# bark-simulator/planner-miqp

Measured on AMD Instinct MI355X. Metric: MIQP solves/sec to 1% gap, 2-agent x 20-step x 32-region, higher is better.
Workload: dtype f64

## Files before the change

planner_miqp_amd/csrc/kernels.hip:

```cpp
#include <hip/hip_runtime.h>

#include "host_inst.hpp"

#ifndef MIQP_RHO
#define MIQP_RHO 1.0e5
#endif

#ifndef MIQP_IPM_WPE
#define MIQP_IPM_WPE 3
#endif

#ifdef MIQP_ABLATE
#define MIQP_ABL (B.abl)
#else
#define MIQP_ABL 0
#endif
namespace miqp {

constexpr double RHO_EL = MIQP_RHO;
constexpr double FEAS_TOL = 1.0e-6;
constexpr double QP_TOL = 1.0e-6;
#ifndef MIQP_T0
#define MIQP_T0 1.0e-3
#endif
// ... 1937 lines not shown
    int nk = 0, nfar = 0, nnear = 0; double fmin_ = 1e300;
    for (int a = 0; a < nalt; ++a) {
      const double cb = objlb + clift[a];
      if (inc_now < 1e300 && (inc_now - cb) <= gapi * (1e-10 + fabs(inc_now))) { if (B.stats) atomicAdd(&B.stats[56], 1ull); continue; }
      int negm = 0;
      if (chosen.kind == 3 && ck[a] >= 0 && ck[a] < N && (B.seq_kinds & 0x10000) == 0) {
        negm = 1 << (int)comp[base + ck[a] * stride];
        for (int a2 = 1; a2 < a; ++a2) if (ck[a2] == ck[a]) negm |= 1 << ca[a2];
      }
      const bool tf = (cb - cst) > thr && B.batch_depth[node] != REPAIR_ROOT;
      k_ck[nk] = ck[a]; k_ca[nk] = ca[a]; k_neg[nk] = negm; k_ord[nk] = a; k_bnd[nk] = cb - cst;
      k_pos[nk] = tf ? (0x40000000 | nfar++) : nnear++;
      if (tf) fmin_ = fmin(fmin_, cb - cst);
      nk++;
    }
    int fbase = 0, obase = 0, ob2 = 0, extra2 = 0; bool okalloc = true;
    if (nnear > 0) {
      obase = atomicAdd(&B.open_count[inst], nnear);
      if (obase + nnear > B.open_cap) {
        for (int q = obase; q < obase + nnear && q < B.open_cap; ++q) { size_t oi = ((size_t)B.open_sel * B.n_slots + slot) * B.open_cap + q; B.open_bound[oi] = 1e300; B.open_node[oi] = -1; B.open_depth[oi] = 0; }
        if (B.far_cap > 0) { for (int q = 0; q < nk; ++q) if (!(k_pos[q] & 0x40000000)) { k_pos[q] = 0x40000000 | nfar++; fmin_ = fmin(fmin_, k_bnd[q]); } }
        else okalloc = false;
        nnear = 0; obase = 0;
      }
    }
    const int nnear_kept = nnear;
    if (nfar > 0) {
      fbase = atomicAdd(&B.far_count[inst], nfar);
      if (fbase + nfar <= B.far_cap) atomicMin(&B.far_minkey[inst], d2key(fmin_));
      else {
        for (int q = fbase; q < fbase + nfar && q < B.far_cap; ++q) { B.far_bound[(size_t)slot * B.far_cap + q] = 1e300; B.far_node[(size_t)slot * B.far_cap + q] = -1; }
        int extra = 0;
        for (int q = 0; q < nk; ++q) if (k_pos[q] & 0x40000000) k_pos[q] = 0x20000000 | extra++;
        nfar = 0;
        ob2 = atomicAdd(&B.open_count[inst], extra); extra2 = extra;
        if (ob2 + extra > B.open_cap) {
          okalloc = false;
          for (int q = ob2; q < ob2 + extra && q < B.open_cap; ++q) { size_t oi = ((size_t)B.open_sel * B.n_slots + slot) * B.open_cap + q; B.open_bound[oi] = 1e300; B.open_node[oi] = -1; B.open_depth[oi] = 0; }
        }
        sh_base[3] = ob2;
      }
    }
    if (okalloc && nk > 0) {
      unsigned int h = atomicAdd(B.free_head, (unsigned int)nk);
      if ((int)(*B.free_limit - h) >= nk) {
        for (int q = 0; q < nk; ++q) slots[q] = B.free_q[(h + q) % (unsigned int)B.pool_cap];
      } else {
        int nb = atomicAdd(B.pool_count, nk);
        if (nb + nk > B.pool_cap) okalloc = false;
        for (int q = 0; q < nk; ++q) slots[q] = nb + q;
      }
    }
    if (!okalloc) {
      atomicOr(&B.inst_flags[inst], 1);
      for (int q = fbase; q < fbase + nfar; ++q) { B.far_bound[(size_t)slot * B.far_cap + q] = 1e300; B.far_node[(size_t)slot * B.far_cap + q] = -1; }
      for (int q = obase; q < obase + nnear_kept && q < B.open_cap; ++q) { size_t oi = ((size_t)B.open_sel * B.n_slots + slot) * B.open_cap + q; B.open_bound[oi] = 1e300; B.open_node[oi] = -1; B.open_depth[oi] = 0; }
      for (int q = ob2; q < ob2 + extra2 && q < B.open_cap; ++q) { size_t oi = ((size_t)B.open_sel * B.n_slots + slot) * B.open_cap + q; B.open_bound[oi] = 1e300; B.open_node[oi] = -1; B.open_depth[oi] = 0; }
      nk = 0;
    }
    if (B.stats && nk > 0) { atomicAdd(&B.stats[43], 1ull); atomicAdd(&B.stats[44], (unsigned long long)nk); atomicAdd(&B.stats[48 + chosen.kind], 1ull); atomicAdd(&B.stats[52 + chosen.kind], (unsigned long long)nk); }
    sh_base[0] = fbase; sh_base[1] = obase; sh_base[2] = nk;
  }
  __syncthreads();
  PROF_T(te5);
  const int nk = sh_base[2];
  if (nk <= 0) { FREE_NODE(); return; }
  {
    for (int q = 0; q < nk; ++q) {
      signed char* dst = B.pool_fix + (size_t)slots[q] * Y.fixlen;
      const int kk = k_ck[q]; const signed char av = (signed char)k_ca[q];
      int negidx = -1; const int negm = k_neg[q];
      if (chosen.kind == 3 && kk >= 0 && kk < N && (B.seq_kinds & 0x10000) == 0) negidx = Y.f_c2n + (chosen.c * N + kk) * 4 + chosen.o;
      if (kk != -2) {
        for (int k8 = lane; k8 < Y.fixlen / 8; k8 += 64) ((unsigned long long*)cfix)[k8] = ((const unsigned long long*)fix)[k8];
        __syncthreads();
        for (int j = jlo + lane; j <= jhi; j += 64) { const int k = base + j * stride; if (fix[k] < 0) { if (j < kk) cfix[k] = comp[k]; else if (j == kk) cfix[k] = av; } }
        __syncthreads();
        if (lane == 0 && negidx >= 0) cfix[negidx] = (signed char)negm;
        __syncthreads();
        for (int k8 = lane; k8 < Y.fixlen / 8; k8 += 64) ((unsigned long long*)dst)[k8] = ((const unsigned long long*)cfix)[k8];
        __syncthreads();
      } else
      for (int k = lane; k < Y.fixlen; k += 64) {
        signed char v = fix[k];
        int rel = k - base;
        if (v < 0 && rel >= 0 && rel % stride == 0) {
          int j = rel / stride;
          if (j >= jlo && j <= jhi) { if (j < kk) v = comp[k]; else if (j == kk) v = av; }
        }
        if (k == negidx) v = (signed char)negm;
        if (kk == -2) {
          v = (fix[k] < 0 && k < Y.f_c2n) ? comp[k] : fix[k];
          if ((B.opt2 & 0x10000) && fix[k] < 0 && k >= Y.f_env && k < Y.f_c2c && (k - Y.f_env) % 5 != 0) v = fix[k];
          if (B.probe_margin > 0.0 && fix[k] < 0 && ploose[k]) v = fix[k];
        }
        dst[k] = v;
      }
      if (B.pool_origin && lane == 0) {
        int cls = k_ord[q] > 0 ? 1 : 0;
        if (chosen.kind == 0 && cls) { const int rq = (int)comp[base + chosen.i * stride] >> 2, cq = k_ca[q] >> 2; const int dq = T[Y.i_regj + chosen.c * P + cq] - T[Y.i_regj + chosen.c * P + rq]; const int ad = abs(dq) % Y.R;
          cls = (k_ca[q] & 3) == 3 ? 3 : ((ad == 1 || ad == Y.R - 1) ? 1 : 2); }
        B.pool_origin[slots[q]] = (signed char)(kk == -2 ? 15 : 4 * chosen.kind + cls);
      }
    }
    if (B.pool_big && lane < nk) B.pool_big[slots[lane]] = pumped ? (unsigned char)((((big_parent >> 4) + 1) << 4) | 1) : (unsigned char)(big_parent & ~12);
    if (B.pool_Z) {
      for (int q = 0; q < nk; ++q) { if (slots[q] >= B.z_cap) continue; double* zd = B.pool_Z + (size_t)slots[q] * N * NZ; for (int k = lane; k < N * NZ; k += 64) zd[k] = Z[k]; }
    }
    if (B.pool_A) {
      const bool as_node = B.batch_A && B.batch_large && B.batch_large[node] <= 1;
      const unsigned short av_ = as_node ? B.batch_A[(size_t)node * 64 + lane] : (unsigned short)0xFFFFu;
      for (int q = 0; q < nk; ++q) { if (slots[q] >= B.z_cap) continue; B.pool_A[(size_t)slots[q] * 64 + lane] = av_; }
      if (B.ring_M && lane < nk && slots[lane] < B.z_cap) B.pool_Mtag[slots[lane]] = as_node ? B.batch_Mtag[node] : 0ull;
    }
    if (lane < nk) {
      int pd = B.batch_depth[node] >> 6;
      int pref = k_ord[lane];
      if (B.opt2 & 2) {
        pref = 0;
        for (int q = 0; q < nk; ++q) if (k_bnd[q] < k_bnd[lane] || (k_bnd[q] == k_bnd[lane] && q < lane)) pref++;
      }
      const int dw = k_ck[lane] == -2 ? (((pd + 2) << 6) | 63) : (((pd + 1) << 6) | (62 - (pref < 62 ? pref : 62)));
      if (k_pos[lane] & 0x40000000) {
        size_t oi = (size_t)slot * B.far_cap + sh_base[0] + (k_pos[lane] & 0x3FFFFFFF);
        B.far_bound[oi] = k_bnd[lane]; B.far_node[oi] = slots[lane]; B.far_depth[oi] = dw;
      } else {
        const int np_ = (k_pos[lane] & 0x20000000) ? sh_base[3] + (k_pos[lane] & 0x1FFFFFFF) : sh_base[1] + k_pos[lane];
        size_t oi = ((size_t)B.open_sel * B.n_slots + slot) * B.open_cap + np_;
        B.open_bound[oi] = k_bnd[lane]; B.open_node[oi] = slots[lane]; B.open_depth[oi] = dw;
      }
    }
  }
  FREE_NODE();
#ifdef MIQP_PROFILE
  { PROF_T(te6);
    if (lane == 0) { atomicAdd(&B.prof[100], (unsigned long long)(te1 - te0)); atomicAdd(&B.prof[101], (unsigned long long)(te2 - te1)); atomicAdd(&B.prof[102], (unsigned long long)(te3 - te2));
                     atomicAdd(&B.prof[103], (unsigned long long)(te4 - te3)); atomicAdd(&B.prof[104], (unsigned long long)(te5 - te4)); atomicAdd(&B.prof[105], (unsigned long long)(te6 - te5)); atomicAdd(&B.prof[106], 1ull); } }
#endif
#undef FREE_NODE
}

constexpr int SEL_THREADS = 1024;
constexpr int SEL_LOWSHIFT = 24;

__device__ inline int wave_append(int* counter, bool pred) {
  const unsigned long long mk = __ballot(pred);
  const int lane = threadIdx.x & 63;
  int base = 0;
  if (lane == (int)(__ffsll((long long)mk) - 1)) base = atomicAdd(counter, __popcll(mk));
  base = __shfl(base, mk ? (int)(__ffsll((long long)mk) - 1) : 0);
  return base + __popcll(mk & ((1ull << lane) - 1ull));
}

__global__ void __launch_bounds__(SEL_THREADS) select_kernel(DevBuf B, int round) {
  const Layout& Y = B.Y;
  const int slot = blockIdx.x, tid = threadIdx.x;
#ifdef MIQP_PROFILE
  if (slot == 0 && tid == 0) {
    const unsigned long long a = B.prof[120], b = B.prof[121], c = B.prof[122];
    if (b != 0 && a != ~0ull && a != 0) { B.prof[123] += b - a; B.prof[124] += b - c; B.prof[125] += 1; }
    B.prof[120] = ~0ull; B.prof[121] = 0; B.prof[122] = ~0ull;
  }
#endif
  const int inst = B.slot_inst[slot];
  if (inst < 0 || B.inst_done[inst] || B.inst_kill[inst]) { if (tid == 0) B.slot_demand[slot] = 0; }
  if (inst < 0) return;
  const int cap = B.open_cap;
  __shared__ int sh_take, sh_base, sh_m, sh_keep, sh_pick, sh_ties, sh_w, sh_mv, sh_all, sh_elig;
  __shared__ double sh_inc;
  __shared__ unsigned int hist[256], dhist[256], sh_wsum[4];
  __shared__ int sh_bin;
  __shared__ int sh_dkeep, sh_tiecnt, sh_ndef;
  __shared__ unsigned long long sh_thr2;
  __shared__ unsigned long long sh_prefix, sh_thr, sh_fmin;
  __shared__ double red[SEL_THREADS];
  if (B.inst_done[inst]) return;
  const size_t src = ((size_t)B.open_sel * B.n_slots + slot) * cap, dst = ((size_t)(1 - B.open_sel) * B.n_slots + slot) * cap;
  unsigned long long* keys = B.open_key + (size_t)slot * cap;
  PROF_T(ts0);
  if (tid == 0) {
    unsigned long long key = B.inc_key[inst];
    sh_inc = inc_from_key(key);
    sh_take = -1;
    sh_thr = key != B.inc_seen[inst] ? key : ~0ull;
    sh_fmin = ~0ull;
    sh_m = 0; sh_keep = 0; sh_pick = 0; sh_ties = 0; sh_ndef = 0;
  }
  __syncthreads();
  if (sh_thr != ~0ull) {
    const unsigned long long key = sh_thr;
    const int pbc = B.prev_bc < B.batch_cap ? B.prev_bc : B.batch_cap;
    for (int k = tid; k < pbc; k += SEL_THREADS) if (B.batch_candkey[k] == key && B.batch_candinst[k] == inst) atomicMin(&sh_fmin, d2key(B.batch_obj[k]));
    __syncthreads();
    const unsigned long long bo = sh_fmin;
    if (tid == 0) sh_dkeep = 0x7FFFFFFF;
    __syncthreads();
    if (bo != ~0ull) for (int k = tid; k < pbc; k += SEL_THREADS) if (B.batch_candkey[k] == key && B.batch_candinst[k] == inst && d2key(B.batch_obj[k]) == bo) atomicMin(&sh_dkeep, k);
    __syncthreads();
    if (tid == 0 && sh_dkeep != 0x7FFFFFFF) { sh_take = sh_dkeep; B.inc_seen[inst] = key; }
  }
  __syncthreads();
  if (sh_take >= 0) {
    const int bslot = sh_take;
    const signed char* cf = B.batch_comp + (size_t)bslot * Y.fixlen; signed char* df = B.inc_fix + (size_t)inst * Y.fixlen;
    for (int k = tid; k < Y.fixlen; k += SEL_THREADS) df[k] = cf[k];
    const double* zs = B.batch_Z + (size_t)bslot * Y.N * Y.nz; double* zd = B.inc_Z + (size_t)inst * Y.N * Y.nz;
    for (int k = tid; k < Y.N * Y.nz; k += SEL_THREADS) zd[k] = zs[k];
    if (B.inc_A && B.batch_A && B.batch_Mtag) {
      if (tid < 64) B.inc_A[(size_t)inst * 64 + tid] = B.batch_A[(size_t)bslot * 64 + tid];
      if (tid == 0) B.inc_Mtag[inst] = B.batch_Mtag[bslot];
    }
    if (tid == 0) { B.inc_obj[inst] = B.batch_obj[bslot]; if (B.inst_lns) B.inst_lns[inst] |= 1; }
  }
  __syncthreads();
  if (B.inst_kill[inst]) {
    int nn = B.open_count[inst]; if (nn > cap) nn = cap;
    for (int k = tid; k < nn; k += SEL_THREADS) { const int nd = B.open_node[src + k]; if (nd >= 0) { unsigned int q_ = atomicAdd(B.free_tail, 1u); B.free_q[q_ % (unsigned int)B.pool_cap] = nd; } }
    int fn = B.far_cap > 0 ? B.far_count[inst] : 0; if (fn > B.far_cap) fn = B.far_cap;
    for (int k = tid; k < fn; k += SEL_THREADS) { const int nd = B.far_node[(size_t)slot * (size_t)B.far_cap + k]; if (nd >= 0) { unsigned int q_ = atomicAdd(B.free_tail, 1u); B.free_q[q_ % (unsigned int)B.pool_cap] = nd; } }
    __syncthreads();
    if (tid == 0) {
      B.open_count[inst] = 0; if (B.far_cap > 0) B.far_count[inst] = 0;
      atomicOr(&B.inst_flags[inst], 2); B.inst_done[inst] = 1; atomicSub(B.active_insts, 1);
    }
    return;
  }
  PROF_T(ts1);
  const double inc = fmin(sh_inc < 1e300 ? B.inc_obj[inst] : 1e300, B.inc_ext[inst]);
  const double cst = B.inst_const[inst];
  const double gap = B.inst_gap[inst];
  int n = B.open_count[inst]; if (n > cap) n = cap;
  auto prunable = [&](double b) { return inc < 1e300 && (inc - (b + cst)) <= gap * (1e-10 + fabs(inc)); };
  auto radix = [&](auto keyf, int cnt, int need) -> int {
    if (tid == 0) { sh_prefix = 0ull; sh_all = 0; }
    __syncthreads();
    for (int shift = 56; shift >= SEL_LOWSHIFT; shift -= 8) {
      if (tid < 256) hist[tid] = 0u;
      __syncthreads();
      const unsigned long long prefix = sh_prefix;
      const unsigned long long himask = shift == 56 ? 0ull : (~0ull << (shift + 8));
      for (int k = tid; k < cnt; k += SEL_THREADS) {
        unsigned long long key = keyf(k);
        if (key != ~0ull && (key & himask) == prefix) atomicAdd(&hist[(key >> shift) & 255ull], 1u);
      }
      __syncthreads();
      if (tid == 0) sh_bin = 256;
      unsigned int hv = 0, hx = 0;
      if (tid < 256) {
        hv = hist[tid]; hx = hv;
#pragma unroll
        for (int o = 1; o < 64; o <<= 1) { const unsigned int y = __shfl_up(hx, o); if ((tid & 63) >= o) hx += y; }
        if ((tid & 63) == 63) sh_wsum[tid >> 6] = hx;
      }
      __syncthreads();
      if (tid < 256) {
#pragma unroll
        for (int w = 0; w < 3; ++w) if (w < (tid >> 6)) hx += sh_wsum[w];
        if (hx >= (unsigned int)need) atomicMin(&sh_bin, tid);
        if (tid == 255) sh_wsum[3] = hx;
      }
      __syncthreads();
      {
        const int bin0 = sh_bin;
        if (tid == (bin0 < 256 ? bin0 : 255)) {
          const int bin = bin0 < 256 ? bin0 : 255;
          const unsigned int cum = bin0 < 256 ? hx - hv : sh_wsum[3];
          if (bin0 >= 256 && shift == 56) sh_all = 1;
          sh_prefix = prefix | ((unsigned long long)bin << shift);
          sh_pick = need - (int)cum;
          sh_tiecnt = (int)hv;
        }
      }
      __syncthreads();
      need = sh_pick;
      if (sh_all) break;
    }
    __syncthreads();
    return need;
  };
  const unsigned long long lowmask = (1ull << SEL_LOWSHIFT) - 1ull;
  int keep = cap / 4; { const int k2 = 2 * B.batch_cap > 65536 ? 2 * B.batch_cap : 65536; if (keep > k2) keep = k2; }
  const int spill_at = 2 * keep;
  const size_t fb = (size_t)slot * (size_t)B.far_cap;
  int fc = B.far_cap > 0 ? B.far_count[inst] : 0; if (fc > B.far_cap) fc = B.far_cap;
  const int dive_every = (B.seq_kinds >> 18) & 3;
  const bool periodic = dive_every == 0 ? (round & 3) == 3 : (dive_every == 1 ? false : (dive_every == 2 ? (round & 7) == 7 : (round & 1) == 1));
  bool pool_tight;
  { const int pc = *B.pool_count; const long long live = (long long)(pc < B.pool_cap ? pc : B.pool_cap) - (long long)(int)(*B.free_tail - *B.free_head);
    pool_tight = live > (long long)B.pool_cap / 10 * 9; }
  const bool lists_full = B.far_cap > 0 ? fc > B.far_cap / 4 * 3 : n > cap / 2;
  const bool dive = !(inc < 1e300) || periodic || lists_full || pool_tight;
  auto order_key = [&](double b, int dp) -> unsigned long long {
    const int dbias = (B.seq_kinds >> 24) & 3;
    const double bb = dbias ? b - (dbias == 1 ? 1e-4 : (dbias == 2 ? 1e-3 : 1e-2)) * fabs(b) * (double)(dp >> 6) : b;
    if (dive) { const unsigned long long kd = ((unsigned long long)(0xFFFF - (dp < 0xFFFF ? dp : 0xFFFF)) << 48) | (d2key(fmax(b, -1e300)) >> 16); return kd == ~0ull ? ~0ull - 1 : kd; }
    const double kv = fmax(bb, -1e300);
    const unsigned long long key = d2key(kv); return key == ~0ull ? ~0ull - 1 : key;
  };
  PROF_T(ts2);
  for (int k = tid; k < 256; k += SEL_THREADS) dhist[k] = 0u;
  __syncthreads();
  double lb = 1e300; int mloc = 0, ndef = 0;
  const bool big_round = B.probe_every <= 1 || (round % B.probe_every) == B.probe_every - 1;
  for (int k = tid; k < n; k += SEL_THREADS) {
    double b = B.open_bound[src + k]; int nd = B.open_node[src + k]; int dp = B.open_depth[src + k];
    unsigned long long key = ~0ull;
    if (nd < 0) { keys[k] = key; continue; }
    if (prunable(b)) {
      unsigned int q_ = atomicAdd(B.free_tail, 1u); B.free_q[q_ % (unsigned int)B.pool_cap] = nd;
    } else {
      lb = fmin(lb, b);
      key = order_key(b, dp);
      if (!big_round && is_probe_word(dp)) { key = ~0ull - 1; ndef++; }
      atomicAdd(&dhist[(dp >> 6) > 255 ? 255 : (dp >> 6)], 1u);
      mloc++;
    }
    keys[k] = key;
  }
  if (mloc) atomicAdd(&sh_m, mloc);
  if (ndef) atomicAdd(&sh_ndef, ndef);
  __syncthreads();
  int m = sh_m;
  PROF_T(ts3);
  if (fc > 0 && m < keep / 4 && cap - n >= 64) {
    auto fkey = [&](int k) -> unsigned long long {
      const double b = B.far_bound[fb + k];
      if (B.far_node[fb + k] < 0 || prunable(b)) return ~0ull;
      const unsigned long long key = d2key(b); return key == ~0ull ? ~0ull - 1 : key;
    };
    int stride = fc > 4 * keep ? (fc + keep - 1) / keep : 1;
    if (stride > 1 && (fc + stride - 1) / stride > cap - n) stride = (fc + (cap - n) - 1) / (cap - n);
    if (stride > 1) {
      const int ns = (fc + stride - 1) / stride;
      for (int j = tid; j < ns; j += SEL_THREADS) keys[n + j] = fkey(j * stride);
      __syncthreads();
      int need_s = (keep - m) / stride; if (need_s < 1) need_s = 1;
      radix([&](int k) { return keys[n + k]; }, ns, need_s);
    } else radix(fkey, fc, keep - m);
    const unsigned long long thr = sh_all ? ~0ull : sh_prefix;
    if (tid == 0) { sh_w = 0; sh_mv = 0; sh_fmin = ~0ull; }
    __syncthreads();
    int room = cap - n; if (room > keep - m) room = keep - m; if (room < 0) room = 0;
    constexpr int PER = 4;
    for (int c0 = 0; c0 < fc; c0 += SEL_THREADS * PER) {
      double eb[PER]; int en[PER], ed[PER], act[PER];
#pragma unroll
      for (int j = 0; j < PER; ++j) {
        const int k = c0 + j * SEL_THREADS + tid;
        act[j] = -1;
        if (k < fc) {
          eb[j] = B.far_bound[fb + k]; en[j] = B.far_node[fb + k]; ed[j] = B.far_depth[fb + k];
          if (en[j] < 0) act[j] = -1;
          else if (prunable(eb[j])) act[j] = 0;
          else { unsigned long long key = d2key(eb[j]); if (key == ~0ull) key = ~0ull - 1; act[j] = ((key & ~lowmask) <= thr) ? 2 : 1; }
        }
      }
      __syncthreads();
#pragma unroll
      for (int j = 0; j < PER; ++j) {
        if (act[j] == 0) { unsigned int q_ = atomicAdd(B.free_tail, 1u); B.free_q[q_ % (unsigned int)B.pool_cap] = en[j]; }
        int t = wave_append(&sh_mv, act[j] == 2);
        if (act[j] == 2) {
          if (t < room) {
            B.open_bound[src + n + t] = eb[j]; B.open_node[src + n + t] = en[j]; B.open_depth[src + n + t] = ed[j]; keys[n + t] = order_key(eb[j], ed[j]);
            lb = fmin(lb, eb[j]); atomicAdd(&dhist[(ed[j] >> 6) > 255 ? 255 : (ed[j] >> 6)], 1u);
          } else act[j] = 1;
        }
        int pos = wave_append(&sh_w, act[j] == 1);
        if (act[j] == 1) { B.far_bound[fb + pos] = eb[j]; B.far_node[fb + pos] = en[j]; B.far_depth[fb + pos] = ed[j]; atomicMin(&sh_fmin, d2key(eb[j])); }
      }
      __syncthreads();
    }
    const int moved = sh_mv < room ? sh_mv : room;
    n += moved; m += moved;
    fc = sh_w;
    __syncthreads();
    if (tid == 0) {
      B.far_count[inst] = fc; B.far_minkey[inst] = sh_fmin;
      B.near_thr[inst] = (fc > 0 && thr != ~0ull) ? key2d(thr | lowmask) : 1e300;
    }
  }
  PROF_T(ts4);
  lb = wave_min(lb);
  __syncthreads();
  if ((tid & 63) == 0) red[tid >> 6] = lb;
  __syncthreads();
#pragma unroll
  for (int w = 0; w < SEL_THREADS / 64; ++w) lb = fmin(lb, red[w]);
  if (fc > 0) lb = fmin(lb, key2d(B.far_minkey[inst]));
  const bool spill = B.far_cap > 0 && m > spill_at && fc < B.far_cap;
  unsigned long long thr_spill = ~0ull;
  if (spill) {
    radix([&](int k) { return keys[k]; }, n, keep);
    thr_spill = sh_all ? ~0ull : sh_prefix;
    if (tid == 0) { unsigned int cum = 0; int d = 255; for (; d >= 0; --d) { if (cum + dhist[d] > (unsigned int)(keep / 2)) break; cum += dhist[d]; } sh_dkeep = d + 1; }
    __syncthreads();
  }
  const int dkeep = sh_dkeep;
  PROF_T(ts5);
  if (tid == 0) sh_pick = 0;
  __syncthreads();
  const int act_now = *B.active_insts;
  const int focus_at = 16 << ((B.seq_kinds >> 29) & 3);
  const bool focus = act_now <= focus_at && inc < 1e300 && (B.seq_kinds & 0x8000000) == 0;
  if (focus) {
    const double gme = (inc - (lb + cst)) / (1e-10 + fabs(inc));
    int cntl = 0;
    for (int sj = tid; sj < B.n_slots; sj += SEL_THREADS) {
      const int j = B.slot_inst[sj];
      if (j < 0 || j == inst || B.inst_done[j]) continue;
      const double ij = B.inc_obj[j];
      const double gj = ij < 1e299 ? (ij - B.lower_bound[j]) / (1e-10 + fabs(ij)) : 1e300;
      if (gj < gme || (gj == gme && j < inst)) cntl++;
    }
    if (cntl) atomicAdd(&sh_pick, cntl);
  }
  __syncthreads();
  const int rank = sh_pick;
  __syncthreads();
  int m_elig = m - sh_ndef;
  if (!dive && inc < 1e300 && B.window_pct < 100 && m > 0) {
    const double top = inc - gap * (1e-10 + fabs(inc)) - cst;
    const double thrw = lb + 0.01 * (double)B.window_pct * fmax(0.0, top - lb);
    const unsigned long long kw = d2key(thrw);
    if (tid == 0) sh_elig = 0;
    __syncthreads();
    int ce = 0;
    for (int k = tid; k < n; k += SEL_THREADS) { const unsigned long long key = keys[k]; if (key != ~0ull && key <= kw) ce++; }
    if (ce) atomicAdd(&sh_elig, ce);
    __syncthreads();
    m_elig = sh_elig < 1 ? 1 : sh_elig;
    if (m_elig > m - sh_ndef) m_elig = m - sh_ndef;
  }
  if (tid == 0) {
    sh_pick = 0;
    int act = act_now; if (act < 1) act = 1;
    int w;
    if (B.seq_kinds & 0x40000000) {
      w = (focus && !(B.seq_kinds & 0x10000000)) ? (B.batch_cap >> (rank + 1 < 30 ? rank + 1 : 30)) : B.batch_cap / act;
      if (w < B.nodes_per_round) w = B.nodes_per_round;
    } else { w = B.slot_take[slot]; if (w < B.base_take && !(B.young_nodes > 0 && B.inst_nodes[inst] >= (long long)B.young_nodes)) w = B.base_take; }
    if (B.width_cap > 0 && w > B.width_cap) w = B.width_cap;
    if (!(inc < 1e300) && w > 512) w = 512;
    if (B.lns_narrow > 0 && B.inst_lns && (B.inst_lns[inst] & 1) && inc < 1e300 && B.inst_nodes[inst] >= (long long)B.lns_min_nodes && w > B.lns_narrow) w = B.lns_narrow;
    B.slot_demand[slot] = inc < 1e300 ? m_elig : (m < 512 ? m : 512);
    int take = m_elig < w ? m_elig : w;
    const int maxch = B.far_cap > 0 ? 8 : 64;
    int room = (cap - m) / maxch; if (room < 1) room = 1;
    if (B.far_cap > 0 && room < 1024) room = 1024;
    if (take > room) take = room;
    int base = take > 0 ? atomicAdd(B.batch_count, take) : 0;
    if (base + take > B.batch_cap) take = B.batch_cap > base ? B.batch_cap - base : 0;
    sh_take = take; sh_base = base;
    double lbt = ((n > 0 || fc > 0) && lb < 1e300 ? lb + cst : inc);
    if (inc < 1e300 && lbt > inc) lbt = inc;
    B.lower_bound[inst] = lbt;
    if (m == 0 && fc == 0) { B.inst_done[inst] = 1; atomicSub(B.active_insts, 1); }
    B.inst_mode[inst] = dive ? 1 : 0;
    sh_thr = ~0ull; sh_w = fc; sh_fmin = ~0ull;
  }
  __syncthreads();
  PROF_T(ts6);
  const int take = sh_take, base = sh_base;
  auto second_key = [&](unsigned long long key, int dp) -> unsigned long long { return (((key & lowmask) << 6) | (unsigned long long)(63 - (dp & 63))) << 34; };
  if (take > 0 && take < m) {
    int need = radix([&](int k) { return keys[k]; }, n, take);
    const unsigned long long thr1 = sh_prefix; const int tiecnt = sh_tiecnt;
    __syncthreads();
    unsigned long long thr2 = ~0ull;
    if (B.det_ties && need < tiecnt) {
      if (tiecnt <= SEL_THREADS) {
        unsigned long long* tie = (unsigned long long*)red;
        if (tid == 0) sh_elig = 0;
        __syncthreads();
        for (int k = tid; k < n; k += SEL_THREADS) {
          const unsigned long long key = keys[k];
          if (key != ~0ull && (key & ~lowmask) == thr1) { const int t = atomicAdd(&sh_elig, 1); if (t < SEL_THREADS) tie[t] = second_key(key, B.open_depth[src + k]); }
        }
        __syncthreads();
        const int tc = sh_elig < SEL_THREADS ? sh_elig : SEL_THREADS;
        if (tid < tc) {
          const unsigned long long v = tie[tid]; int lt = 0, le = 0;
          for (int j = 0; j < tc; ++j) { const unsigned long long u = tie[j]; lt += u < v ? 1 : 0; le += u <= v ? 1 : 0; }
          if (lt < need && need <= le) { sh_thr2 = v; sh_ties = need - lt; }
        }
        __syncthreads();
        thr2 = sh_thr2; need = sh_ties;
        __syncthreads();
      } else {
        need = radix([&](int k) -> unsigned long long { const unsigned long long key = keys[k]; if (key == ~0ull || (key & ~lowmask) != thr1) return ~0ull; return second_key(key, B.open_depth[src + k]); }, n, need);
        thr2 = sh_prefix;
        __syncthreads();
      }
    }
    if (tid == 0) { sh_thr = thr1; sh_thr2 = thr2; sh_ties = need; sh_pick = 0; }
    __syncthreads();
  } else if (tid == 0) { sh_thr = take >= m ? ~0ull : 0ull;    sh_thr2 = ~0ull; sh_ties = 0x7FFFFFFF; sh_pick = 0; }
  __syncthreads();
  PROF_T(ts7);
  const unsigned long long thr = sh_thr, thr2 = sh_thr2;
  for (int k0 = 0; k0 < n; k0 += SEL_THREADS) {
    const int k = k0 + tid;
    unsigned long long key = k < n ? keys[k] : ~0ull;
    const bool live = key != ~0ull;
    double b = 0.0; int nd = 0, dp = 0;
    bool pick = false;
    if (live) {
      b = B.open_bound[src + k]; nd = B.open_node[src + k]; dp = B.open_depth[src + k];
      if (take > 0) {
        const unsigned long long kh = key & (~0ull << SEL_LOWSHIFT);
        if (kh < thr) pick = true;
        else if (kh == thr) {
          const unsigned long long s2 = thr2 != ~0ull ? second_key(key, dp) : 0ull;
          if (thr2 != ~0ull && s2 < thr2) pick = true;
          else if (thr2 == ~0ull || s2 == thr2) { int t = atomicAdd(&sh_ties, -1); pick = t > 0; }
        }
      }
      if (pick) {
        int pos = atomicAdd(&sh_pick, 1);
        if (pos < take) { B.batch_node[base + pos] = nd; B.batch_inst[base + pos] = inst; B.batch_bound[base + pos] = b; B.batch_depth[base + pos] = dp;
                          if (B.batch_large) { const int lc_ = large_class(B, nd, dp, inc < 1e300); B.batch_large[base + pos] = (unsigned char)lc_;
                            if (lc_ && B.cls_list) { const int q_ = atomicAdd(&B.cls_count[lc_ - 1], 1); if (q_ < B.batch_cap) B.cls_list[(size_t)(lc_ - 1) * B.batch_cap + q_] = base + pos; } } }
        else pick = false;
      }
    }
    bool tofar = live && !pick && spill && (key & ~lowmask) > thr_spill && (dp >> 6) < dkeep;
    int fpos = wave_append(&sh_w, tofar);
    if (tofar) {
      if (fpos < B.far_cap) { B.far_bound[fb + fpos] = b; B.far_node[fb + fpos] = nd; B.far_depth[fb + fpos] = dp; atomicMin(&sh_fmin, d2key(b)); }
      else tofar = false;
    }
    const bool stay = live && !pick && !tofar;
    int pos = wave_append(&sh_keep, stay);
    if (stay) { B.open_bound[dst + pos] = b; B.open_node[dst + pos] = nd; B.open_depth[dst + pos] = dp; }
  }
  __syncthreads();
  if (tid == 0) {
    B.open_count[inst] = sh_keep;
    if (spill) {
      B.far_count[inst] = sh_w < B.far_cap ? sh_w : B.far_cap;
      if (sh_fmin != ~0ull) atomicMin(&B.far_minkey[inst], sh_fmin);
      B.near_thr[inst] = dive ? -1e300 : (thr_spill != ~0ull ? key2d(thr_spill | lowmask) : 1e300);
    }
  }
#ifdef MIQP_PROFILE
  { PROF_T(ts8);
    if (tid == 0) { const long long tt[9] = {ts0, ts1, ts2, ts3, ts4, ts5, ts6, ts7, ts8};
      for (int q = 0; q < 8; ++q) atomicAdd(&B.prof[110 + q], (unsigned long long)(tt[q + 1] - tt[q]));
      atomicAdd(&B.prof[118], 1ull); atomicAdd(&B.prof[119], (unsigned long long)n); } }
#endif
}

__global__ void admit_kernel(DevBuf B, const int* pairs, int n, int sel) {
  const int k = blockIdx.x * blockDim.x + threadIdx.x;
  if (k >= n) return;
  const int slot = pairs[2 * k], inst = pairs[2 * k + 1];
  const int old = B.slot_inst[slot];
  if (old >= 0) B.inst_slot[old] = -1;
  B.slot_inst[slot] = inst;
  if (inst < 0) return;
  B.inst_slot[inst] = slot;
  const int nr = B.root_cnt[inst];
  const size_t base = ((size_t)sel * B.n_slots + slot) * B.open_cap;
  for (int r = 0; r < nr; ++r) { B.open_bound[base + r] = -1e300; B.open_node[base + r] = B.root_node[(size_t)inst * B.root_stride + r]; B.open_depth[base + r] = B.root_depth[(size_t)inst * B.root_stride + r]; }
  B.open_count[inst] = nr;
  atomicAdd(B.active_insts, 1);
}

__global__ void __launch_bounds__(1024) share_kernel(DevBuf B) {
  __shared__ long long red[1024];
  __shared__ int sh_lo, sh_hi;
  const int tid = threadIdx.x, NSL = B.n_slots;
  const int WCAP = NSL == 1 ? (B.batch_cap > 8192 ? B.batch_cap : 8192) : 8192;
  auto bsum = [&](long long v) -> long long {
#pragma unroll
    for (int o = 32; o > 0; o >>= 1) v += __shfl_xor(v, o);
    __syncthreads();
    if ((tid & 63) == 0) red[tid >> 6] = v;
    __syncthreads();
    long long t = 0;
#pragma unroll
    for (int w = 0; w < 16; ++w) t += red[w];
    return t;
  };
  const long long target = (long long)B.batch_cap - (long long)B.batch_cap / 16;
  int base = B.base_take;
  if (B.floor_pct > 0) {
    if (tid == 0) { sh_lo = B.base_take; sh_hi = B.share_cap; }
    __syncthreads();
    const long long budget = target * B.floor_pct / 100;
    for (int itn = 0; itn < 12; ++itn) {
      const int lo = sh_lo, hi = sh_hi;
      if (lo >= hi) break;
      const int mid = lo + (hi - lo + 1) / 2;
      long long a = 0;
      for (int k = tid; k < NSL; k += 1024) { const int d = B.slot_demand[k]; a += d < mid ? d : mid; }
      const long long tot = bsum(a);
      if (tid == 0) { if (tot <= budget) sh_lo = mid; else sh_hi = mid - 1; }
      __syncthreads();
    }
    base = sh_lo;
    __syncthreads();
  }
  auto base_of = [&](int k) -> int {
    const int d = B.slot_demand[k], inst = B.slot_inst[k];
    if (B.young_nodes > 0 && inst >= 0 && B.inst_nodes[inst] >= (long long)B.young_nodes) return 0;
    return d < base ? d : base;
  };
  long long ab = 0;
  for (int k = tid; k < NSL; k += 1024) ab += base_of(k);
  const long long SB = bsum(ab);
  const long long rest = target - SB;
  const long long cap = B.share_cap;
  auto more_of = [&](int k) -> long long {
    const int d = B.slot_demand[k]; const long long c = d < cap ? d : cap;
    const int b = base_of(k);
    return c > b ? c - b : 0;
  };
  constexpr int SH_SLOTS = 2048;
  __shared__ int s_inst[SH_SLOTS]; __shared__ long long s_more[SH_SLOTS];
  const bool staged = NSL <= SH_SLOTS;
  if (staged) { for (int k = tid; k < NSL; k += 1024) { s_inst[k] = B.slot_inst[k]; s_more[k] = more_of(k); } }
  __syncthreads();
  long long at = 0;
  for (int k = tid; k < NSL; k += 1024) {
    const int inst = staged ? s_inst[k] : B.slot_inst[k];
    int take = base_of(k);
    const long long more = staged ? s_more[k] : more_of(k);
    if (inst >= 0 && more > 0 && rest > 0) {
      long long before = 0;
      if (staged) { for (int j = 0; j < NSL; ++j) { const int ij = s_inst[j]; if (ij >= 0 && ij < inst) before += s_more[j]; } }
      else { for (int j = 0; j < NSL; ++j) { const int ij = B.slot_inst[j]; if (ij >= 0 && ij < inst) before += more_of(j); } }
      long long ex = rest - before; if (ex > more) ex = more;
      if (ex > 0) take += (int)ex;
    }
    B.slot_take[k] = take; at += take;
  }
  const long long left = target - bsum(at);
  if (left <= 0) return;
  if (tid == 0) { sh_lo = 0; sh_hi = WCAP; }
  __syncthreads();
  for (int itn = 0; itn < 16; ++itn) {
    const int lo = sh_lo, hi = sh_hi;
    if (lo >= hi) break;
    const int mid = lo + (hi - lo + 1) / 2;
    long long a = 0;
    for (int k = tid; k < NSL; k += 1024) { long long r = (long long)B.slot_demand[k] - B.slot_take[k]; if (r > WCAP - B.slot_take[k]) r = WCAP - B.slot_take[k]; a += r < mid ? (r > 0 ? r : 0) : mid; }
    const long long tot = bsum(a);
    if (tid == 0) { if (tot <= left) sh_lo = mid; else sh_hi = mid - 1; }
    __syncthreads();
  }
  const int L = sh_lo;
  for (int k = tid; k < NSL; k += 1024) {
    long long r = (long long)B.slot_demand[k] - B.slot_take[k]; if (r > WCAP - B.slot_take[k]) r = WCAP - B.slot_take[k];
    if (r > 0) B.slot_take[k] += (int)(r < L ? r : L);
  }
}

constexpr int LNS_MAX = 512;
__global__ void __launch_bounds__(64) lns_kernel(DevBuf B) {
  const Layout& Y = B.Y;
  const int slot = blockIdx.x, lane = threadIdx.x;
  const int inst = B.slot_inst[slot];
  if (inst < 0) return;
  const int flags = B.inst_lns[inst];
  const bool want_skel = (B.lns_mode & 32) && !(flags & 2) && Y.NP > 0;
  if (!(flags & 1) && !want_skel) return;
  if (B.inst_nodes[inst] < (long long)B.lns_min_nodes) return;
  if ((flags & 1) && !want_skel && B.lns_step > 0.0) {
    const double io = B.inc_obj[inst] + B.inst_const[inst], last = B.inst_lns_obj[inst];
    if (last < 1e299 && io > last - B.lns_step * fabs(last)) return;
  }
  __shared__ int nb_c[LNS_MAX], nb_i[LNS_MAX], nb_n[LNS_MAX], nb_code[LNS_MAX];
  __shared__ int nb_c2[LNS_MAX], nb_n2[LNS_MAX], nb_code2[LNS_MAX];
  __shared__ int nb_rec[LNS_MAX];
  __shared__ int sh_n, sh_base, sh_rec, sh_skel;
  const int N = Y.N, C = Y.C;
  const signed char* inc = B.inc_fix + (size_t)inst * Y.fixlen;
  if (lane == 0) {
    int n = 0;
    auto push = [&](int first, int stride, int cnt, int val) { if (n < LNS_MAX) { nb_c[n] = first; nb_i[n] = stride; nb_n[n] = cnt; nb_code[n] = val; nb_n2[n] = 0; n++; } };
    const bool alive = !B.inst_done[inst] && !B.inst_kill[inst];
    sh_skel = 0;
    if (alive && want_skel) {
      sh_skel = 1;
      const int* T = B.inst_i + (size_t)inst * Y.istride;
      for (int p = 0; p < Y.NP; ++p) {
// ... 168 lines not shown
```

Measured before the change: 1089.

## Batch select-kernel loads per thread and skip radix passes via key range

Adds a sel_walk helper so each thread issues four independent global loads before consuming them, and uses it for every scan loop in select_kernel. The open-list scan now tracks the min and max of the order keys, reduced across the block, and the radix select starts at the first byte where they differ instead of always at the top byte. Both aim to cut memory latency stalls and redundant histogram passes. In exchange the loops clamp out-of-range indices to n-1, which adds a few extra loads and register pressure, and the radix prefix and sh_all logic becomes harder to verify.

```diff
diff --git a/planner_miqp_amd/csrc/kernels.hip b/planner_miqp_amd/csrc/kernels.hip
--- a/planner_miqp_amd/csrc/kernels.hip
+++ b/planner_miqp_amd/csrc/kernels.hip
@@ -2113,6 +2113,32 @@
   return base + __popcll(mk & ((1ull << lane) - 1ull));
 }
 
+constexpr int SEL_PER = 4;
+template <class LD, class USE>
+__device__ inline void sel_walk(int n, LD ld, USE use) {
+  const int tid = threadIdx.x;
+  for (int c0 = 0; c0 < n; c0 += SEL_THREADS * SEL_PER) {
+    decltype(ld(0)) v[SEL_PER];
+#pragma unroll
+    for (int j = 0; j < SEL_PER; ++j) { const int k = c0 + j * SEL_THREADS + tid; v[j] = ld(k < n ? k : n - 1); }
+#pragma unroll
+    for (int j = 0; j < SEL_PER; ++j) { const int k = c0 + j * SEL_THREADS + tid; if (k < n) use(k, v[j]); }
+  }
+}
+struct SelEntry { double b; int nd, dp; };
+struct SelKeyDepth { unsigned long long key; int dp; };
+struct SelCand { unsigned long long key; int inst; double obj; };
+__device__ inline unsigned long long wave_min_u64(unsigned long long v) {
+#pragma unroll
+  for (int o = 32; o > 0; o >>= 1) { const unsigned long long u = __shfl_xor(v, o); v = u < v ? u : v; }
+  return v;
+}
+__device__ inline unsigned long long wave_max_u64(unsigned long long v) {
+#pragma unroll
+  for (int o = 32; o > 0; o >>= 1) { const unsigned long long u = __shfl_xor(v, o); v = u > v ? u : v; }
+  return v;
+}
+
 __global__ void __launch_bounds__(SEL_THREADS) select_kernel(DevBuf B, int round) {
   const Layout& Y = B.Y;
   const int slot = blockIdx.x, tid = threadIdx.x;
@@ -2151,12 +2177,13 @@
   if (sh_thr != ~0ull) {
     const unsigned long long key = sh_thr;
     const int pbc = B.prev_bc < B.batch_cap ? B.prev_bc : B.batch_cap;
-    for (int k = tid; k < pbc; k += SEL_THREADS) if (B.batch_candkey[k] == key && B.batch_candinst[k] == inst) atomicMin(&sh_fmin, d2key(B.batch_obj[k]));
+    auto cand = [&](int k) { return SelCand{B.batch_candkey[k], B.batch_candinst[k], B.batch_obj[k]}; };
+    sel_walk(pbc, cand, [&](int, const SelCand& c) { if (c.key == key && c.inst == inst) atomicMin(&sh_fmin, d2key(c.obj)); });
     __syncthreads();
     const unsigned long long bo = sh_fmin;
     if (tid == 0) sh_dkeep = 0x7FFFFFFF;
     __syncthreads();
-    if (bo != ~0ull) for (int k = tid; k < pbc; k += SEL_THREADS) if (B.batch_candkey[k] == key && B.batch_candinst[k] == inst && d2key(B.batch_obj[k]) == bo) atomicMin(&sh_dkeep, k);
+    if (bo != ~0ull) sel_walk(pbc, cand, [&](int k, const SelCand& c) { if (c.key == key && c.inst == inst && d2key(c.obj) == bo) atomicMin(&sh_dkeep, k); });
     __syncthreads();
     if (tid == 0 && sh_dkeep != 0x7FFFFFFF) { sh_take = sh_dkeep; B.inc_seen[inst] = key; }
   }
@@ -2176,9 +2203,10 @@
   __syncthreads();
   if (B.inst_kill[inst]) {
     int nn = B.open_count[inst]; if (nn > cap) nn = cap;
-    for (int k = tid; k < nn; k += SEL_THREADS) { const int nd = B.open_node[src + k]; if (nd >= 0) { unsigned int q_ = atomicAdd(B.free_tail, 1u); B.free_q[q_ % (unsigned int)B.pool_cap] = nd; } }
+    auto give_back = [&](int, int nd) { if (nd >= 0) { unsigned int q_ = atomicAdd(B.free_tail, 1u); B.free_q[q_ % (unsigned int)B.pool_cap] = nd; } };
+    sel_walk(nn, [&](int k) { return B.open_node[src + k]; }, give_back);
     int fn = B.far_cap > 0 ? B.far_count[inst] : 0; if (fn > B.far_cap) fn = B.far_cap;
-    for (int k = tid; k < fn; k += SEL_THREADS) { const int nd = B.far_node[(size_t)slot * (size_t)B.far_cap + k]; if (nd >= 0) { unsigned int q_ = atomicAdd(B.free_tail, 1u); B.free_q[q_ % (unsigned int)B.pool_cap] = nd; } }
+    sel_walk(fn, [&](int k) { return B.far_node[(size_t)slot * (size_t)B.far_cap + k]; }, give_back);
     __syncthreads();
     if (tid == 0) {
       B.open_count[inst] = 0; if (B.far_cap > 0) B.far_count[inst] = 0;
@@ -2192,18 +2220,24 @@
   const double gap = B.inst_gap[inst];
   int n = B.open_count[inst]; if (n > cap) n = cap;
   auto prunable = [&](double b) { return inc < 1e300 && (inc - (b + cst)) <= gap * (1e-10 + fabs(inc)); };
-  auto radix = [&](auto keyf, int cnt, int need) -> int {
-    if (tid == 0) { sh_prefix = 0ull; sh_all = 0; }
+  auto radix = [&](auto ld, auto keyf, int cnt, int need, unsigned long long kmn, unsigned long long kmx) -> int {
+    int start = 56;
+    if (kmn <= kmx) {
+      const unsigned long long x = kmn ^ kmx;
+      start = x ? ((63 - __clzll((long long)x)) & ~7) : SEL_LOWSHIFT;
+      if (start < SEL_LOWSHIFT) start = SEL_LOWSHIFT;
+    }
+    if (tid == 0) { sh_prefix = start == 56 ? 0ull : (kmn & (~0ull << (start + 8))); sh_all = 0; }
     __syncthreads();
-    for (int shift = 56; shift >= SEL_LOWSHIFT; shift -= 8) {
+    for (int shift = start; shift >= SEL_LOWSHIFT; shift -= 8) {
       if (tid < 256) hist[tid] = 0u;
       __syncthreads();
       const unsigned long long prefix = sh_prefix;
       const unsigned long long himask = shift == 56 ? 0ull : (~0ull << (shift + 8));
-      for (int k = tid; k < cnt; k += SEL_THREADS) {
-        unsigned long long key = keyf(k);
+      sel_walk(cnt, ld, [&](int, const auto& v) {
+        const unsigned long long key = keyf(v);
         if (key != ~0ull && (key & himask) == prefix) atomicAdd(&hist[(key >> shift) & 255ull], 1u);
-      }
+      });
       __syncthreads();
       if (tid == 0) sh_bin = 256;
       unsigned int hv = 0, hx = 0;
@@ -2226,8 +2260,9 @@
         if (tid == (bin0 < 256 ? bin0 : 255)) {
           const int bin = bin0 < 256 ? bin0 : 255;
           const unsigned int cum = bin0 < 256 ? hx - hv : sh_wsum[3];
-          if (bin0 >= 256 && shift == 56) sh_all = 1;
-          sh_prefix = prefix | ((unsigned long long)bin << shift);
+          const bool all = bin0 >= 256 && shift == start;
+          if (all) sh_all = 1;
+          sh_prefix = all ? 255ull << 56 : prefix | ((unsigned long long)bin << shift);
           sh_pick = need - (int)cum;
           sh_tiecnt = (int)hv;
         }
@@ -2263,41 +2298,59 @@
   __syncthreads();
   double lb = 1e300; int mloc = 0, ndef = 0;
   const bool big_round = B.probe_every <= 1 || (round % B.probe_every) == B.probe_every - 1;
-  for (int k = tid; k < n; k += SEL_THREADS) {
-    double b = B.open_bound[src + k]; int nd = B.open_node[src + k]; int dp = B.open_depth[src + k];
+  unsigned long long kmn = ~0ull, kmx = 0ull;
+  sel_walk(n, [&](int k) { return SelEntry{B.open_bound[src + k], B.open_node[src + k], B.open_depth[src + k]}; }, [&](int k, const SelEntry& e) {
+    const double b = e.b; const int nd = e.nd, dp = e.dp;
     unsigned long long key = ~0ull;
-    if (nd < 0) { keys[k] = key; continue; }
+    if (nd < 0) { keys[k] = key; return; }
     if (prunable(b)) {
       unsigned int q_ = atomicAdd(B.free_tail, 1u); B.free_q[q_ % (unsigned int)B.pool_cap] = nd;
     } else {
       lb = fmin(lb, b);
       key = order_key(b, dp);
       if (!big_round && is_probe_word(dp)) { key = ~0ull - 1; ndef++; }
+      kmn = key < kmn ? key : kmn; kmx = key > kmx ? key : kmx;
       atomicAdd(&dhist[(dp >> 6) > 255 ? 255 : (dp >> 6)], 1u);
       mloc++;
     }
     keys[k] = key;
-  }
+  });
   if (mloc) atomicAdd(&sh_m, mloc);
   if (ndef) atomicAdd(&sh_ndef, ndef);
   __syncthreads();
   int m = sh_m;
+  auto key_range = [&](unsigned long long& mn, unsigned long long& mx) {
+    unsigned long long* rk = (unsigned long long*)red;
+    mn = wave_min_u64(mn); mx = wave_max_u64(mx);
+    __syncthreads();
+    if ((tid & 63) == 0) { rk[SEL_THREADS / 64 + (tid >> 6)] = mn; rk[2 * (SEL_THREADS / 64) + (tid >> 6)] = mx; }
+    __syncthreads();
+#pragma unroll
+    for (int w = 0; w < SEL_THREADS / 64; ++w) {
+      const unsigned long long a = rk[SEL_THREADS / 64 + w], b = rk[2 * (SEL_THREADS / 64) + w];
+      mn = a < mn ? a : mn; mx = b > mx ? b : mx;
+    }
+  };
   PROF_T(ts3);
   if (fc > 0 && m < keep / 4 && cap - n >= 64) {
-    auto fkey = [&](int k) -> unsigned long long {
-      const double b = B.far_bound[fb + k];
-      if (B.far_node[fb + k] < 0 || prunable(b)) return ~0ull;
-      const unsigned long long key = d2key(b); return key == ~0ull ? ~0ull - 1 : key;
+    auto fld = [&](int k) { return SelEntry{B.far_bound[fb + k], B.far_node[fb + k], 0}; };
+    auto fkey = [&](const SelEntry& e) -> unsigned long long {
+      if (e.nd < 0 || prunable(e.b)) return ~0ull;
+      const unsigned long long key = d2key(e.b); return key == ~0ull ? ~0ull - 1 : key;
     };
     int stride = fc > 4 * keep ? (fc + keep - 1) / keep : 1;
     if (stride > 1 && (fc + stride - 1) / stride > cap - n) stride = (fc + (cap - n) - 1) / (cap - n);
     if (stride > 1) {
       const int ns = (fc + stride - 1) / stride;
-      for (int j = tid; j < ns; j += SEL_THREADS) keys[n + j] = fkey(j * stride);
-      __syncthreads();
+      unsigned long long smn = ~0ull, smx = 0ull;
+      sel_walk(ns, [&](int j) { return fld(j * stride); }, [&](int j, const SelEntry& e) {
+        const unsigned long long key = fkey(e); keys[n + j] = key;
+        if (key != ~0ull) { smn = key < smn ? key : smn; smx = key > smx ? key : smx; }
+      });
+      key_range(smn, smx);
       int need_s = (keep - m) / stride; if (need_s < 1) need_s = 1;
-      radix([&](int k) { return keys[n + k]; }, ns, need_s);
-    } else radix(fkey, fc, keep - m);
+      radix([&](int k) { return keys[n + k]; }, [](unsigned long long key) { return key; }, ns, need_s, smn, smx);
+    } else radix(fld, fkey, fc, keep - m, 0ull, ~0ull);
     const unsigned long long thr = sh_all ? ~0ull : sh_prefix;
     if (tid == 0) { sh_w = 0; sh_mv = 0; sh_fmin = ~0ull; }
     __syncthreads();
@@ -2323,7 +2376,9 @@
         int t = wave_append(&sh_mv, act[j] == 2);
         if (act[j] == 2) {
           if (t < room) {
-            B.open_bound[src + n + t] = eb[j]; B.open_node[src + n + t] = en[j]; B.open_depth[src + n + t] = ed[j]; keys[n + t] = order_key(eb[j], ed[j]);
+            const unsigned long long key = order_key(eb[j], ed[j]);
+            B.open_bound[src + n + t] = eb[j]; B.open_node[src + n + t] = en[j]; B.open_depth[src + n + t] = ed[j]; keys[n + t] = key;
+            kmn = key < kmn ? key : kmn; kmx = key > kmx ? key : kmx;
             lb = fmin(lb, eb[j]); atomicAdd(&dhist[(ed[j] >> 6) > 255 ? 255 : (ed[j] >> 6)], 1u);
           } else act[j] = 1;
         }
@@ -2348,11 +2403,14 @@
   __syncthreads();
 #pragma unroll
   for (int w = 0; w < SEL_THREADS / 64; ++w) lb = fmin(lb, red[w]);
+  key_range(kmn, kmx);
   if (fc > 0) lb = fmin(lb, key2d(B.far_minkey[inst]));
   const bool spill = B.far_cap > 0 && m > spill_at && fc < B.far_cap;
+  auto kld = [&](int k) { return keys[k]; };
+  auto kid = [](unsigned long long key) { return key; };
   unsigned long long thr_spill = ~0ull;
   if (spill) {
-    radix([&](int k) { return keys[k]; }, n, keep);
+    radix(kld, kid, n, keep, kmn, kmx);
     thr_spill = sh_all ? ~0ull : sh_prefix;
     if (tid == 0) { unsigned int cum = 0; int d = 255; for (; d >= 0; --d) { if (cum + dhist[d] > (unsigned int)(keep / 2)) break; cum += dhist[d]; } sh_dkeep = d + 1; }
     __syncthreads();
@@ -2387,7 +2445,7 @@
     if (tid == 0) sh_elig = 0;
     __syncthreads();
     int ce = 0;
-    for (int k = tid; k < n; k += SEL_THREADS) { const unsigned long long key = keys[k]; if (key != ~0ull && key <= kw) ce++; }
+    sel_walk(n, kld, [&](int, unsigned long long key) { if (key != ~0ull && key <= kw) ce++; });
     if (ce) atomicAdd(&sh_elig, ce);
     __syncthreads();
     m_elig = sh_elig < 1 ? 1 : sh_elig;
@@ -2425,7 +2483,8 @@
   const int take = sh_take, base = sh_base;
   auto second_key = [&](unsigned long long key, int dp) -> unsigned long long { return (((key & lowmask) << 6) | (unsigned long long)(63 - (dp & 63))) << 34; };
   if (take > 0 && take < m) {
-    int need = radix([&](int k) { return keys[k]; }, n, take);
+    int need = radix(kld, kid, n, take, kmn, kmx);
+    auto kdld = [&](int k) { return SelKeyDepth{keys[k], B.open_depth[src + k]}; };
     const unsigned long long thr1 = sh_prefix; const int tiecnt = sh_tiecnt;
     __syncthreads();
     unsigned long long thr2 = ~0ull;
@@ -2434,10 +2493,9 @@
         unsigned long long* tie = (unsigned long long*)red;
         if (tid == 0) sh_elig = 0;
         __syncthreads();
-        for (int k = tid; k < n; k += SEL_THREADS) {
-          const unsigned long long key = keys[k];
-          if (key != ~0ull && (key & ~lowmask) == thr1) { const int t = atomicAdd(&sh_elig, 1); if (t < SEL_THREADS) tie[t] = second_key(key, B.open_depth[src + k]); }
-        }
+        sel_walk(n, kdld, [&](int, const SelKeyDepth& e) {
+          if (e.key != ~0ull && (e.key & ~lowmask) == thr1) { const int t = atomicAdd(&sh_elig, 1); if (t < SEL_THREADS) tie[t] = second_key(e.key, e.dp); }
+        });
         __syncthreads();
         const int tc = sh_elig < SEL_THREADS ? sh_elig : SEL_THREADS;
         if (tid < tc) {
@@ -2449,7 +2507,7 @@
         thr2 = sh_thr2; need = sh_ties;
         __syncthreads();
       } else {
-        need = radix([&](int k) -> unsigned long long { const unsigned long long key = keys[k]; if (key == ~0ull || (key & ~lowmask) != thr1) return ~0ull; return second_key(key, B.open_depth[src + k]); }, n, need);
+        need = radix(kdld, [&](const SelKeyDepth& e) -> unsigned long long { return (e.key == ~0ull || (e.key & ~lowmask) != thr1) ? ~0ull : second_key(e.key, e.dp); }, n, need, 0ull, ~0ull);
         thr2 = sh_prefix;
         __syncthreads();
       }
@@ -2460,14 +2518,21 @@
   __syncthreads();
   PROF_T(ts7);
   const unsigned long long thr = sh_thr, thr2 = sh_thr2;
-  for (int k0 = 0; k0 < n; k0 += SEL_THREADS) {
-    const int k = k0 + tid;
-    unsigned long long key = k < n ? keys[k] : ~0ull;
+  for (int c0 = 0; c0 < n; c0 += SEL_THREADS * SEL_PER) {
+   unsigned long long ek[SEL_PER]; SelEntry ee[SEL_PER];
+#pragma unroll
+   for (int j = 0; j < SEL_PER; ++j) {
+     const int k = c0 + j * SEL_THREADS + tid, kc = k < n ? k : n - 1;
+     ek[j] = keys[kc]; ee[j] = SelEntry{B.open_bound[src + kc], B.open_node[src + kc], B.open_depth[src + kc]};
+   }
+#pragma unroll
+   for (int j = 0; j < SEL_PER; ++j) {
+    const int k = c0 + j * SEL_THREADS + tid;
+    const unsigned long long key = k < n ? ek[j] : ~0ull;
     const bool live = key != ~0ull;
-    double b = 0.0; int nd = 0, dp = 0;
+    const double b = ee[j].b; const int nd = ee[j].nd, dp = ee[j].dp;
     bool pick = false;
     if (live) {
-      b = B.open_bound[src + k]; nd = B.open_node[src + k]; dp = B.open_depth[src + k];
       if (take > 0) {
         const unsigned long long kh = key & (~0ull << SEL_LOWSHIFT);
         if (kh < thr) pick = true;
@@ -2494,6 +2559,7 @@
     const bool stay = live && !pick && !tofar;
     int pos = wave_append(&sh_keep, stay);
     if (stay) { B.open_bound[dst + pos] = b; B.open_node[dst + pos] = nd; B.open_depth[dst + pos] = dp; }
+   }
   }
   __syncthreads();
   if (tid == 0) {
```

Result: slower. 1057 (-2.9%).
